# HilaManor/AudioEditingCode

Hardware: AMD Instinct MI355X
Metric: edited-clips/sec (200-step inv+edit, 10 s@16 kHz) (higher is better)
Workload: dtype f32

## Files before the change

audioeditingcode_amd/csrc/attention.hip:

```cpp
#include <mutex>
#include "aed_common.h"

typedef float f32x4 __attribute__((ext_vector_type(4)));

#include "attn_params.h"

#define KV_TILE 64
#define Q_TILE 64

template <int D>
__global__ __launch_bounds__(256) void attention_kernel(AttnParams p) {
    constexpr int KLD = D + 4;
    constexpr int VLD = KV_TILE + 4;
    constexpr int NB = D / 16;
    __shared__ __attribute__((aligned(16))) float Ks[KV_TILE * KLD];
    __shared__ __attribute__((aligned(16))) float Vt[D * VLD];
    __shared__ __attribute__((aligned(16))) float Ps[4 * 16 * VLD];

    const int tid = threadIdx.x;
    const int lane = tid & 63, wave = tid >> 6;
    const int fi = lane & 15, fh = lane >> 4;
    const int b = blockIdx.z, head = blockIdx.y;
    const int q0 = blockIdx.x * Q_TILE + wave * 16;
    const int hoff = head * D;

    const float* Q = p.q + (size_t)b * p.bsq + hoff;
    const float* K = p.k + (size_t)b * p.bsk + hoff;
    const float* V = p.v + (size_t)b * p.bsv + hoff;
    const float* bias = p.bias ? p.bias + (size_t)b * p.ld_bias : nullptr;

    float4 qf[NB];
    {
        const int qr = q0 + fi;
#pragma unroll
        for (int blk = 0; blk < NB; ++blk) {
            qf[blk] = make_float4(0.f, 0.f, 0.f, 0.f);
            if (qr < p.Nq) qf[blk] = *reinterpret_cast<const float4*>(Q + (size_t)qr * p.ldq + 16 * blk + 4 * fh);
        }
    }
    f32x4 oacc[NB];
#pragma unroll
    for (int c = 0; c < NB; ++c) oacc[c] = (f32x4){0.f, 0.f, 0.f, 0.f};
    float m_run[4], l_run[4];
#pragma unroll
    for (int r = 0; r < 4; ++r) { m_run[r] = -INFINITY; l_run[r] = 0.f; }

    float* Pw = Ps + wave * 16 * VLD;

    for (int k0 = 0; k0 < p.Nk; k0 += KV_TILE) {
        for (int idx = tid; idx < KV_TILE * (D / 4); idx += 256) {
            const int key = idx / (D / 4), c4 = idx - key * (D / 4);
            float4 v = make_float4(0.f, 0.f, 0.f, 0.f);
            if (k0 + key < p.Nk) v = *reinterpret_cast<const float4*>(K + (size_t)(k0 + key) * p.ldk + 4 * c4);
            *reinterpret_cast<float4*>(Ks + key * KLD + 4 * c4) = v;
        }
        {
            const int key = tid & 63, dg = tid >> 6;
            for (int dd = dg * 4; dd < D; dd += 16) {
                float4 v = make_float4(0.f, 0.f, 0.f, 0.f);
                if (k0 + key < p.Nk) v = *reinterpret_cast<const float4*>(V + (size_t)(k0 + key) * p.ldv + dd);
                Vt[(dd + 0) * VLD + key] = v.x;
                Vt[(dd + 1) * VLD + key] = v.y;
                Vt[(dd + 2) * VLD + key] = v.z;
                Vt[(dd + 3) * VLD + key] = v.w;
            }
        }
        __syncthreads();

        f32x4 sacc[4];
#pragma unroll
        for (int j = 0; j < 4; ++j) sacc[j] = (f32x4){0.f, 0.f, 0.f, 0.f};
#pragma unroll
        for (int blk = 0; blk < NB; ++blk) {
#pragma unroll
            for (int j = 0; j < 4; ++j) {
                const float4 kf = *reinterpret_cast<const float4*>(Ks + (16 * j + fi) * KLD + 16 * blk + 4 * fh);
                sacc[j] = __builtin_amdgcn_mfma_f32_16x16x4f32(qf[blk].x, kf.x, sacc[j], 0, 0, 0);
                sacc[j] = __builtin_amdgcn_mfma_f32_16x16x4f32(qf[blk].y, kf.y, sacc[j], 0, 0, 0);
                sacc[j] = __builtin_amdgcn_mfma_f32_16x16x4f32(qf[blk].z, kf.z, sacc[j], 0, 0, 0);
                sacc[j] = __builtin_amdgcn_mfma_f32_16x16x4f32(qf[blk].w, kf.w, sacc[j], 0, 0, 0);
            }
        }
        float tmax[4];
#pragma unroll
        for (int r = 0; r < 4; ++r) tmax[r] = -INFINITY;
#pragma unroll
        for (int j = 0; j < 4; ++j) {
            const int key = k0 + 16 * j + fi;
            const bool ok = key < p.Nk;
            const float bv = (ok && bias) ? bias[key] : 0.f;
#pragma unroll
            for (int r = 0; r < 4; ++r) {
                float s = ok ? sacc[j][r] * p.scale + bv : -INFINITY;
                sacc[j][r] = s;
                tmax[r] = fmaxf(tmax[r], s);
            }
        }
#pragma unroll
        for (int r = 0; r < 4; ++r) {
#pragma unroll
            for (int o = 8; o > 0; o >>= 1) tmax[r] = fmaxf(tmax[r], __shfl_xor(tmax[r], o, 16));
        }
        float alpha[4], rsum[4];
#pragma unroll
        for (int r = 0; r < 4; ++r) {
            const float mn = fmaxf(m_run[r], tmax[r]);
            alpha[r] = __expf(m_run[r] - mn);
            m_run[r] = mn;
            rsum[r] = 0.f;
        }
#pragma unroll
        for (int j = 0; j < 4; ++j) {
#pragma unroll
            for (int r = 0; r < 4; ++r) {
                const float pv = __expf(sacc[j][r] - m_run[r]);
                rsum[r] += pv;
                Pw[(4 * fh + r) * VLD + 16 * j + fi] = pv;
            }
        }
#pragma unroll
        for (int r = 0; r < 4; ++r) {
#pragma unroll
            for (int o = 8; o > 0; o >>= 1) rsum[r] += __shfl_xor(rsum[r], o, 16);
            l_run[r] = l_run[r] * alpha[r] + rsum[r];
        }
#pragma unroll
        for (int c = 0; c < NB; ++c)
#pragma unroll
            for (int r = 0; r < 4; ++r) oacc[c][r] *= alpha[r];

        __builtin_amdgcn_fence(__ATOMIC_ACQ_REL, "wavefront");
        __builtin_amdgcn_wave_barrier();

#pragma unroll
        for (int kb = 0; kb < 4; ++kb) {
            const float4 pf = *reinterpret_cast<const float4*>(Pw + fi * VLD + 16 * kb + 4 * fh);
#pragma unroll
            for (int c = 0; c < NB; ++c) {
                const float4 vf = *reinterpret_cast<const float4*>(Vt + (16 * c + fi) * VLD + 16 * kb + 4 * fh);
                oacc[c] = __builtin_amdgcn_mfma_f32_16x16x4f32(pf.x, vf.x, oacc[c], 0, 0, 0);
                oacc[c] = __builtin_amdgcn_mfma_f32_16x16x4f32(pf.y, vf.y, oacc[c], 0, 0, 0);
                oacc[c] = __builtin_amdgcn_mfma_f32_16x16x4f32(pf.z, vf.z, oacc[c], 0, 0, 0);
                oacc[c] = __builtin_amdgcn_mfma_f32_16x16x4f32(pf.w, vf.w, oacc[c], 0, 0, 0);
            }
        }
        __syncthreads();
    }

    float* O = p.o + (size_t)b * p.bso + hoff;
#pragma unroll
    for (int r = 0; r < 4; ++r) {
        const int qr = q0 + 4 * fh + r;
        if (qr >= p.Nq) continue;
        const float inv = 1.0f / l_run[r];
#pragma unroll
        for (int c = 0; c < NB; ++c) O[(size_t)qr * p.ldo + 16 * c + fi] = oacc[c][r] * inv;
    }
}

typedef float f32x16a __attribute__((ext_vector_type(16)));

template <int D, int KSPLIT>
__global__ __launch_bounds__(256) void attention_t_kernel(AttnParams p) {
    constexpr int DT = (D + 31) / 32;
    constexpr int KLD = D + 4;
    constexpr int VLD = 32 + 4;
    constexpr int NJ = D / 8;
    constexpr int SLAB = 32 * KLD + DT * 32 * VLD;
    constexpr int MSZ = DT * 16 + 2;
    static_assert(D % 8 == 0, "head dim");
    extern __shared__ __attribute__((aligned(16))) float smem[];
    const int tid = threadIdx.x, lane = tid & 63, wave = tid >> 6;
    const int fi = lane & 31, fh = lane >> 5;
    float* Ks = smem + wave * SLAB;
    float* Vt = Ks + 32 * KLD;

    int qt, head, b;
    {
        const unsigned nx = gridDim.x, ny = gridDim.y, nwg = nx * ny * gridDim.z;
        const unsigned orig = blockIdx.x + nx * (blockIdx.y + ny * blockIdx.z);
        const unsigned xcd = orig & 7u, q = nwg >> 3, r = nwg & 7u;
        const unsigned id = (xcd < r ? xcd * (q + 1) : r * (q + 1) + (xcd - r) * q) + (orig >> 3);
        qt = (int)(id % nx);
        head = (int)((id / nx) % ny);
        b = (int)(id / (nx * ny));
    }
    const int q0 = (KSPLIT == 1 ? qt * 128 + wave * 32 : qt * 32);
    const int hoff = head * D;
    const float* Q = p.q + (size_t)b * p.bsq + hoff;
    const float* K = p.k + (size_t)b * p.bsk + hoff;
    const float* V = p.v + (size_t)b * p.bsv + hoff;
    const float* bias = p.bias ? p.bias + (size_t)b * p.ld_bias : nullptr;

    float4 qf[NJ];
    {
        const int qr = min(q0 + fi, p.Nq - 1);
#pragma unroll
        for (int j = 0; j < NJ; ++j) {
            float4 v = *reinterpret_cast<const float4*>(Q + (size_t)qr * p.ldq + 8 * j + 4 * fh);
            qf[j] = make_float4(v.x * p.scale, v.y * p.scale, v.z * p.scale, v.w * p.scale);
        }
    }
    f32x16a oacc[DT];
#pragma unroll
    for (int c = 0; c < DT; ++c)
#pragma unroll
        for (int r = 0; r < 16; ++r) oacc[c][r] = 0.f;
    float m_run = -INFINITY, l_run = 0.f;

    constexpr int KC4 = D / 4;
    constexpr int NKL = (32 * KC4) / 64;
    float4 kreg[NKL], vreg[NKL];
    const int ntiles = (p.Nk + 31) / 32;
    auto prefetch = [&](int t) {
        const int k0 = min(t, ntiles - 1) * 32;
#pragma unroll
        for (int i = 0; i < NKL; ++i) {
            const int idx = lane + 64 * i;
            const int key = min(k0 + idx / KC4, p.Nk - 1);
            kreg[i] = *reinterpret_cast<const float4*>(K + (size_t)key * p.ldk + 4 * (idx % KC4));
        }
        const int vk = min(k0 + fi, p.Nk - 1);
#pragma unroll
        for (int i = 0; i < NKL; ++i)
            vreg[i] = *reinterpret_cast<const float4*>(V + (size_t)vk * p.ldv + 4 * (2 * i + fh));
    };
    auto stage = [&]() {
#pragma unroll
        for (int i = 0; i < NKL; ++i) {
            const int idx = lane + 64 * i;
            const float4 v = kreg[i];
            *reinterpret_cast<float4*>(Ks + (idx / KC4) * KLD + 4 * (idx % KC4)) = make_float4(v.x, v.y, v.z, v.w);
        }
#pragma unroll
        for (int i = 0; i < NKL; ++i) {
            const int dd = 4 * (2 * i + fh);
            const float4 v = vreg[i];
            Vt[(dd + 0) * VLD + fi] = v.x;
            Vt[(dd + 1) * VLD + fi] = v.y;
            Vt[(dd + 2) * VLD + fi] = v.z;
            Vt[(dd + 3) * VLD + fi] = v.w;
        }
    };
    if constexpr (DT * 32 > D) {
        for (int e = lane; e < (DT * 32 - D) * VLD; e += 64) Vt[D * VLD + e] = 0.f;
    }

    const int t_first = (KSPLIT == 1 ? 0 : wave);
    constexpr int TSTEP = (KSPLIT == 1 ? 1 : KSPLIT);
    prefetch(t_first);
    for (int t = t_first; t < ntiles; t += TSTEP) {
        stage();
        prefetch(t + TSTEP);
        asm volatile("" ::: "memory");
        __builtin_amdgcn_wave_barrier();
        f32x16a sacc;
#pragma unroll
        for (int r = 0; r < 16; ++r) sacc[r] = 0.f;
#pragma unroll
        for (int j = 0; j < NJ; ++j) {
            const float4 kf = *reinterpret_cast<const float4*>(Ks + fi * KLD + 8 * j + 4 * fh);
            sacc = __builtin_amdgcn_mfma_f32_32x32x2f32(kf.x, qf[j].x, sacc, 0, 0, 0);
            sacc = __builtin_amdgcn_mfma_f32_32x32x2f32(kf.y, qf[j].y, sacc, 0, 0, 0);
            sacc = __builtin_amdgcn_mfma_f32_32x32x2f32(kf.z, qf[j].z, sacc, 0, 0, 0);
            sacc = __builtin_amdgcn_mfma_f32_32x32x2f32(kf.w, qf[j].w, sacc, 0, 0, 0);
        }
        const int k0 = t * 32;
        if (bias) {
#pragma unroll
            for (int rq = 0; rq < 4; ++rq)
#pragma unroll
                for (int e = 0; e < 4; ++e)
                    sacc[4 * rq + e] += bias[min(k0 + 8 * rq + 4 * fh + e, p.Nk - 1)];
        }
        if (k0 + 32 > p.Nk) {
#pragma unroll
            for (int r = 0; r < 16; ++r)
                if (k0 + (r & 3) + 8 * (r >> 2) + 4 * fh >= p.Nk) sacc[r] = -INFINITY;
        }
        float mx = sacc[0];
#pragma unroll
        for (int r = 1; r < 16; ++r) mx = fmaxf(mx, sacc[r]);
        {
            auto sw = __builtin_amdgcn_permlane32_swap(__float_as_uint(mx), __float_as_uint(mx), false, false);
            mx = fmaxf(__uint_as_float(sw[0]), __uint_as_float(sw[1]));
        }
        const float mn = fmaxf(m_run, mx);
        const float alpha = __expf(m_run - mn);
        m_run = mn;
        float rsum = 0.f;
#pragma unroll
        for (int r = 0; r < 16; ++r) {
            sacc[r] = __expf(sacc[r] - mn);
            rsum += sacc[r];
        }
        l_run = l_run * alpha + rsum;
#pragma unroll
        for (int c = 0; c < DT; ++c)
#pragma unroll
            for (int r = 0; r < 16; ++r) oacc[c][r] *= alpha;
#pragma unroll
        for (int rq = 0; rq < 4; ++rq) {
#pragma unroll
            for (int c = 0; c < DT; ++c) {
                const float4 vf = *reinterpret_cast<const float4*>(Vt + (c * 32 + fi) * VLD + 8 * rq + 4 * fh);
                oacc[c] = __builtin_amdgcn_mfma_f32_32x32x2f32(vf.x, sacc[4 * rq + 0], oacc[c], 0, 0, 0);
                oacc[c] = __builtin_amdgcn_mfma_f32_32x32x2f32(vf.y, sacc[4 * rq + 1], oacc[c], 0, 0, 0);
                oacc[c] = __builtin_amdgcn_mfma_f32_32x32x2f32(vf.z, sacc[4 * rq + 2], oacc[c], 0, 0, 0);
                oacc[c] = __builtin_amdgcn_mfma_f32_32x32x2f32(vf.w, sacc[4 * rq + 3], oacc[c], 0, 0, 0);
            }
        }
        asm volatile("" ::: "memory");
        __builtin_amdgcn_wave_barrier();
    }

    if constexpr (KSPLIT > 1) {
        __syncthreads();
        float* mrg = smem;
        if (wave > 0) {
            float* dst = mrg + ((wave - 1) * 64 + lane) * MSZ;
            dst[0] = m_run;
            dst[1] = l_run;
#pragma unroll
            for (int c = 0; c < DT; ++c)
#pragma unroll
                for (int r = 0; r < 16; ++r) dst[2 + 16 * c + r] = oacc[c][r];
        }
        __syncthreads();
        if (wave > 0) return;
        float mt = m_run;
#pragma unroll
        for (int w = 0; w < KSPLIT - 1; ++w) mt = fmaxf(mt, mrg[(w * 64 + lane) * MSZ]);
        const float a0 = (m_run == -INFINITY) ? 0.f : __expf(m_run - mt);
        l_run *= a0;
#pragma unroll
        for (int c = 0; c < DT; ++c)
#pragma unroll
            for (int r = 0; r < 16; ++r) oacc[c][r] *= a0;
#pragma unroll
        for (int w = 0; w < KSPLIT - 1; ++w) {
            const float* src = mrg + (w * 64 + lane) * MSZ;
            const float mw = src[0];
            const float aw = (mw == -INFINITY) ? 0.f : __expf(mw - mt);
            l_run += src[1] * aw;
#pragma unroll
            for (int c = 0; c < DT; ++c)
#pragma unroll
                for (int r = 0; r < 16; ++r) oacc[c][r] += src[2 + 16 * c + r] * aw;
        }
    }
    {
        auto sw = __builtin_amdgcn_permlane32_swap(__float_as_uint(l_run), __float_as_uint(l_run), false, false);
        l_run = __uint_as_float(sw[0]) + __uint_as_float(sw[1]);
    }
    const float inv = 1.0f / l_run;
    const int qr = q0 + fi;
    if (qr < p.Nq) {
        float* O = p.o + (size_t)b * p.bso + hoff + (size_t)qr * p.ldo;
#pragma unroll
        for (int c = 0; c < DT; ++c)
#pragma unroll
            for (int rq = 0; rq < 4; ++rq) {
                const int d0 = c * 32 + 8 * rq + 4 * fh;
                if (d0 < D)
                    *reinterpret_cast<float4*>(O + d0) = make_float4(oacc[c][4 * rq] * inv, oacc[c][4 * rq + 1] * inv,
                                                                     oacc[c][4 * rq + 2] * inv, oacc[c][4 * rq + 3] * inv);
            }
    }
}

template <int D, int KSPLIT>
static int launch_t(const AttnParams& p, int B, hipStream_t s) {
    constexpr int DT = (D + 31) / 32;
    constexpr int SLAB = 32 * (D + 4) + DT * 32 * 36;
    constexpr int MRG = (KSPLIT - 1) * 64 * (DT * 16 + 2);
    const size_t bytes = sizeof(float) * (4 * SLAB > MRG ? 4 * SLAB : MRG);
    static std::once_flag attr_once;
    static hipError_t attr_rc = hipSuccess;
    std::call_once(attr_once, [&] {
        attr_rc = hipFuncSetAttribute((const void*)attention_t_kernel<D, KSPLIT>,
                                      hipFuncAttributeMaxDynamicSharedMemorySize, (int)bytes);
    });
    AED_CHECK_HIP(attr_rc);
    dim3 grid(aed_cdiv(p.Nq, KSPLIT == 1 ? 128 : 32), p.H, B);
    hipLaunchKernelGGL((attention_t_kernel<D, KSPLIT>), grid, dim3(256), bytes, s, p);
    return 0;
}

int launch_attention(const aed_op* op, hipStream_t s) {
    const int32_t* i = op->i;
    AttnParams p;
    p.q = (const float*)op->p[0]; p.k = (const float*)op->p[1]; p.v = (const float*)op->p[2];
    p.bias = (const float*)op->p[3]; p.o = (float*)op->p[4];
    AED_REQUIRE(p.q && p.k && p.v && p.o, "attention: null pointer");
    p.H = i[1]; p.Nq = i[2]; p.Nk = i[3];
    p.ldq = i[5]; p.ldk = i[6]; p.ldv = i[7]; p.ldo = i[8]; p.ld_bias = i[9];
    p.bsq = i[10]; p.bsk = i[11]; p.bsv = i[12]; p.bso = i[13];
    p.scale = op->f[0];
    AED_REQUIRE(p.ldq % 4 == 0 && p.ldk % 4 == 0 && p.ldv % 4 == 0, "attention: row strides must be multiples of 4");
    AED_REQUIRE(p.Nq > 0 && p.Nk > 0, "attention: empty sequence");
    AED_REQUIRE(p.ldo % 4 == 0, "attention: output row stride must be a multiple of 4");
    if (p.Nk > KV_TILE && i[14] != 1) {
        const long wg_ksplit1 = (long)aed_cdiv(p.Nq, 128) * p.H * i[0];
        const bool ks4 = wg_ksplit1 < 2L * aed_num_cus();
        int rc = 0;
        if (((op->flags & 4) && !ks4) || i[14] == 3) {
            rc = launch_attention_x6(p, i[0], i[4], s);
            if (rc >= 0) return rc;
            AED_REQUIRE(i[14] != 3, "attention: the split-bf16 kernel does not take head dim %d / these operands", i[4]);
        }
        switch (i[4]) {
            case 32: rc = ks4 ? launch_t<32, 4>(p, i[0], s) : launch_t<32, 1>(p, i[0], s); break;
            case 48: rc = ks4 ? launch_t<48, 4>(p, i[0], s) : launch_t<48, 1>(p, i[0], s); break;
            case 64: rc = ks4 ? launch_t<64, 4>(p, i[0], s) : launch_t<64, 1>(p, i[0], s); break;
            case 80: rc = ks4 ? launch_t<80, 4>(p, i[0], s) : launch_t<80, 1>(p, i[0], s); break;
            case 16: rc = ks4 ? launch_t<16, 4>(p, i[0], s) : launch_t<16, 1>(p, i[0], s); break;
            default: AED_REQUIRE(false, "attention: unsupported head dim %d (16/32/48/64/80)", i[4]);
        }
        if (rc) return rc;
        AED_CHECK_HIP(hipGetLastError());
        return 0;
    }
    dim3 grid(aed_cdiv(p.Nq, Q_TILE), p.H, i[0]);
    switch (i[4]) {
        case 16: hipLaunchKernelGGL(attention_kernel<16>, grid, dim3(256), 0, s, p); break;
        case 32: hipLaunchKernelGGL(attention_kernel<32>, grid, dim3(256), 0, s, p); break;
        case 48: hipLaunchKernelGGL(attention_kernel<48>, grid, dim3(256), 0, s, p); break;
        case 64: hipLaunchKernelGGL(attention_kernel<64>, grid, dim3(256), 0, s, p); break;
        case 80: hipLaunchKernelGGL(attention_kernel<80>, grid, dim3(256), 0, s, p); break;
        default: AED_REQUIRE(false, "attention: unsupported head dim %d (16/32/48/64/80)", i[4]);
    }
    AED_CHECK_HIP(hipGetLastError());
    return 0;
}
```

audioeditingcode_amd/csrc/attention_x6.hip:

```cpp
#include "attn_params.h"

typedef __bf16 abf16x8 __attribute__((ext_vector_type(8)));
typedef __bf16 abf16x2 __attribute__((ext_vector_type(2)));
typedef float af32x2 __attribute__((ext_vector_type(2)));
typedef float af32x16 __attribute__((ext_vector_type(16)));

__device__ __forceinline__ void ax6_split_pair(float x0, float x1, unsigned& h, unsigned& m, unsigned& l) {
    h = __builtin_bit_cast(unsigned, __builtin_convertvector((af32x2){x0, x1}, abf16x2));
    float r0 = x0 - __uint_as_float(h << 16);
    float r1 = x1 - __uint_as_float(h & 0xffff0000u);
    asm volatile("" : "+v"(r0), "+v"(r1));
    m = __builtin_bit_cast(unsigned, __builtin_convertvector((af32x2){r0, r1}, abf16x2));
    float q0 = r0 - __uint_as_float(m << 16);
    float q1 = r1 - __uint_as_float(m & 0xffff0000u);
    asm volatile("" : "+v"(q0), "+v"(q1));
    l = __builtin_bit_cast(unsigned, __builtin_convertvector((af32x2){q0, q1}, abf16x2));
}

__device__ __forceinline__ void ax6_split8(const float (&x)[8], abf16x8 (&f)[3]) {
    uint4 h, m, l;
    ax6_split_pair(x[0], x[1], h.x, m.x, l.x);
    ax6_split_pair(x[2], x[3], h.y, m.y, l.y);
    ax6_split_pair(x[4], x[5], h.z, m.z, l.z);
    ax6_split_pair(x[6], x[7], h.w, m.w, l.w);
    f[0] = __builtin_bit_cast(abf16x8, h);
    f[1] = __builtin_bit_cast(abf16x8, m);
    f[2] = __builtin_bit_cast(abf16x8, l);
}

__device__ __forceinline__ void ax6_mfma6(af32x16& acc, const abf16x8 (&a)[3], const abf16x8 (&b)[3]) {
    acc = __builtin_amdgcn_mfma_f32_32x32x16_bf16(a[0], b[2], acc, 0, 0, 0);
    acc = __builtin_amdgcn_mfma_f32_32x32x16_bf16(a[2], b[0], acc, 0, 0, 0);
    acc = __builtin_amdgcn_mfma_f32_32x32x16_bf16(a[1], b[1], acc, 0, 0, 0);
    acc = __builtin_amdgcn_mfma_f32_32x32x16_bf16(a[0], b[1], acc, 0, 0, 0);
    acc = __builtin_amdgcn_mfma_f32_32x32x16_bf16(a[1], b[0], acc, 0, 0, 0);
    acc = __builtin_amdgcn_mfma_f32_32x32x16_bf16(a[0], b[0], acc, 0, 0, 0);
}

template <int D>
__global__ __launch_bounds__(256, 2) void attention_x6_kernel(AttnParams p) {
    constexpr int NDB = D / 16;
    constexpr int DT = (D + 31) / 32;
    constexpr int KQ = NDB * 3 * 64;
    constexpr int VQ = 2 * 3 * DT * 64;
    constexpr int STAGE = KQ + VQ;
    constexpr int C4 = D / 4;
    constexpr int NK = (8 * D + 255) / 256;
    constexpr int NV = (8 * D + 255) / 256;
    static_assert(D % 16 == 0 && 2 * STAGE * 16 <= 65536, "head dim");
    __shared__ uint4 lds[2 * STAGE];

    const int tid = threadIdx.x, lane = tid & 63, wave = tid >> 6;
    const int fi = lane & 31, fh = lane >> 5;
    int qt, head, b;
    {
        const unsigned nx = gridDim.x, ny = gridDim.y, nwg = nx * ny * gridDim.z;
        const unsigned orig = blockIdx.x + nx * (blockIdx.y + ny * blockIdx.z);
        const unsigned xcd = orig & 7u, q = nwg >> 3, r = nwg & 7u;
        const unsigned id = (xcd < r ? xcd * (q + 1) : r * (q + 1) + (xcd - r) * q) + (orig >> 3);
        qt = (int)(id % nx);
        head = (int)((id / nx) % ny);
        b = (int)(id / (nx * ny));
    }
    const int q0 = qt * 128 + wave * 32;
    const int hoff = head * D;
    const float* Q = p.q + (size_t)b * p.bsq + hoff;
    const float* K = p.k + (size_t)b * p.bsk + hoff;
    const float* V = p.v + (size_t)b * p.bsv + hoff;
    const float* bias = p.bias ? p.bias + (size_t)b * p.ld_bias : nullptr;

    abf16x8 qp[NDB][3];
    {
        const float* qrow = Q + (size_t)min(q0 + fi, p.Nq - 1) * p.ldq + 8 * fh;
#pragma unroll
        for (int db = 0; db < NDB; ++db) {
            const float4 a = *reinterpret_cast<const float4*>(qrow + 16 * db);
            const float4 c = *reinterpret_cast<const float4*>(qrow + 16 * db + 4);
            const float x[8] = {a.x * p.scale, a.y * p.scale, a.z * p.scale, a.w * p.scale,
                                c.x * p.scale, c.y * p.scale, c.z * p.scale, c.w * p.scale};
            ax6_split8(x, qp[db]);
        }
    }
    af32x16 oacc[DT];
#pragma unroll
    for (int c = 0; c < DT; ++c)
#pragma unroll
        for (int r = 0; r < 16; ++r) oacc[c][r] = 0.f;
    float m_run = -INFINITY, l_run = 0.f;

    const int ntiles = (p.Nk + 31) / 32;
    float4 kreg[2][NK];
    float vreg[2][NV][4];
    auto prefetch = [&](int t, float4 (&kr)[NK], float (&vr)[NV][4]) {
        const int k0 = min(t, ntiles - 1) * 32;
#pragma unroll
        for (int i = 0; i < NK; ++i) {
            const int item = min(tid + 256 * i, 8 * D - 1);
            const int key = min(k0 + item / C4, p.Nk - 1);
            kr[i] = *reinterpret_cast<const float4*>(K + (size_t)key * p.ldk + 4 * (item % C4));
        }
#pragma unroll
        for (int i = 0; i < NV; ++i) {
            const int item = min(tid + 256 * i, 8 * D - 1);
            const int kg = item / D, d = item - kg * D;
#pragma unroll
            for (int j = 0; j < 4; ++j)
                vr[i][j] = V[(size_t)min(k0 + 4 * kg + j, p.Nk - 1) * p.ldv + d];
        }
    };
    auto stage_write = [&](uint4* st, const float4 (&kr)[NK], const float (&vr)[NV][4]) {
        uint2* k2 = reinterpret_cast<uint2*>(st);
        uint2* v2 = reinterpret_cast<uint2*>(st + KQ);
#pragma unroll
        for (int i = 0; i < NK; ++i) {
            const int item = tid + 256 * i;
            if (8 * D % 256 != 0 && item >= 8 * D) break;
            const int key = item / C4, c4 = item % C4;
            unsigned h0, m0, l0, h1, m1, l1;
            ax6_split_pair(kr[i].x, kr[i].y, h0, m0, l0);
            ax6_split_pair(kr[i].z, kr[i].w, h1, m1, l1);
            uint2* dst = k2 + ((c4 >> 2) * 3 * 32 + key) * 4 + ((c4 >> 1) & 1) * 2 + (c4 & 1);
            dst[0] = make_uint2(h0, h1);
            dst[32 * 4] = make_uint2(m0, m1);
            dst[2 * 32 * 4] = make_uint2(l0, l1);
        }
#pragma unroll
        for (int i = 0; i < NV; ++i) {
            const int item = tid + 256 * i;
            if (8 * D % 256 != 0 && item >= 8 * D) break;
            const int kg = item / D, d = item - kg * D;
            unsigned h0, m0, l0, h1, m1, l1;
            ax6_split_pair(vr[i][0], vr[i][1], h0, m0, l0);
            ax6_split_pair(vr[i][2], vr[i][3], h1, m1, l1);
            const int kb = kg >> 2, g = kg & 3;
            uint2* dst = v2 + (((kb * 3) * DT + (d >> 5)) * 32 + (d & 31)) * 4 + (g & 1) * 2 + (g >> 1);
            dst[0] = make_uint2(h0, h1);
            dst[DT * 32 * 4] = make_uint2(m0, m1);
            dst[2 * DT * 32 * 4] = make_uint2(l0, l1);
        }
    };
    if constexpr (DT * 32 > D) {
        for (int e = tid; e < 2 * STAGE; e += 256) lds[e] = make_uint4(0u, 0u, 0u, 0u);
        __syncthreads();
    }

    prefetch(0, kreg[0], vreg[0]);
    prefetch(1, kreg[1], vreg[1]);
    stage_write(lds, kreg[0], vreg[0]);
    prefetch(2, kreg[0], vreg[0]);
    __syncthreads();
    for (int t0 = 0; t0 < ntiles; t0 += 2) {
#pragma unroll
        for (int u = 0; u < 2; ++u) {
            const int t = t0 + u;
            const uint4* st = lds + u * STAGE;
            af32x16 sacc;
#pragma unroll
            for (int r = 0; r < 16; ++r) sacc[r] = 0.f;
#pragma unroll
            for (int db = 0; db < NDB; ++db) {
                abf16x8 kf[3];
#pragma unroll
                for (int pl = 0; pl < 3; ++pl) kf[pl] = __builtin_bit_cast(abf16x8, st[((db * 3 + pl) * 32 + fi) * 2 + fh]);
                ax6_mfma6(sacc, kf, qp[db]);
            }
            stage_write(lds + (u ^ 1) * STAGE, kreg[u ^ 1], vreg[u ^ 1]);
            prefetch(t + 3, kreg[u ^ 1], vreg[u ^ 1]);
            const int k0 = t * 32;
            if (bias) {
#pragma unroll
                for (int rq = 0; rq < 4; ++rq)
#pragma unroll
                    for (int e = 0; e < 4; ++e)
                        sacc[4 * rq + e] += bias[min(k0 + 8 * rq + 4 * fh + e, p.Nk - 1)];
            }
            if (k0 + 32 > p.Nk) {
#pragma unroll
                for (int r = 0; r < 16; ++r)
                    if (k0 + (r & 3) + 8 * (r >> 2) + 4 * fh >= p.Nk) sacc[r] = -INFINITY;
            }
            float mx = sacc[0];
#pragma unroll
            for (int r = 1; r < 16; ++r) mx = fmaxf(mx, sacc[r]);
            {
                auto sw = __builtin_amdgcn_permlane32_swap(__float_as_uint(mx), __float_as_uint(mx), false, false);
                mx = fmaxf(__uint_as_float(sw[0]), __uint_as_float(sw[1]));
            }
            const float mn = fmaxf(m_run, mx);
            const float alpha = __expf(m_run - mn);
            m_run = mn;
            float rsum = 0.f;
#pragma unroll
            for (int r = 0; r < 16; ++r) {
                sacc[r] = __expf(sacc[r] - mn);
                rsum += sacc[r];
            }
            l_run = l_run * alpha + rsum;
#pragma unroll
            for (int c = 0; c < DT; ++c)
#pragma unroll
                for (int r = 0; r < 16; ++r) oacc[c][r] *= alpha;
#pragma unroll
            for (int kb = 0; kb < 2; ++kb) {
                abf16x8 pf[3];
                const float x[8] = {sacc[8 * kb], sacc[8 * kb + 1], sacc[8 * kb + 2], sacc[8 * kb + 3],
                                    sacc[8 * kb + 4], sacc[8 * kb + 5], sacc[8 * kb + 6], sacc[8 * kb + 7]};
                ax6_split8(x, pf);
#pragma unroll
                for (int c = 0; c < DT; ++c) {
                    abf16x8 vf[3];
#pragma unroll
                    for (int pl = 0; pl < 3; ++pl)
                        vf[pl] = __builtin_bit_cast(abf16x8, st[KQ + (((kb * 3 + pl) * DT + c) * 32 + fi) * 2 + fh]);
                    ax6_mfma6(oacc[c], vf, pf);
                }
            }
            __syncthreads();
        }
    }

    {
        auto sw = __builtin_amdgcn_permlane32_swap(__float_as_uint(l_run), __float_as_uint(l_run), false, false);
        l_run = __uint_as_float(sw[0]) + __uint_as_float(sw[1]);
    }
    const float inv = 1.0f / l_run;
    const int qr = q0 + fi;
    if (qr < p.Nq) {
        float* O = p.o + (size_t)b * p.bso + hoff + (size_t)qr * p.ldo;
#pragma unroll
        for (int c = 0; c < DT; ++c)
#pragma unroll
            for (int rq = 0; rq < 4; ++rq) {
                const int d0 = c * 32 + 8 * rq + 4 * fh;
                if (d0 < D)
                    *reinterpret_cast<float4*>(O + d0) = make_float4(oacc[c][4 * rq] * inv, oacc[c][4 * rq + 1] * inv,
                                                                     oacc[c][4 * rq + 2] * inv, oacc[c][4 * rq + 3] * inv);
            }
    }
}

template <int D>
static int launch_ax6(const AttnParams& p, int B, hipStream_t s) {
    dim3 grid(aed_cdiv(p.Nq, 128), p.H, B);
    hipLaunchKernelGGL((attention_x6_kernel<D>), grid, dim3(256), 0, s, p);
    AED_CHECK_HIP(hipGetLastError());
    return 0;
}

int launch_attention_x6(const AttnParams& p, int B, int D, hipStream_t s) {
    if (((uintptr_t)p.q | (uintptr_t)p.k) % 16 != 0) return -1;
    switch (D) {
        case 32: return launch_ax6<32>(p, B, s);
        case 48: return launch_ax6<48>(p, B, s);
        case 64: return launch_ax6<64>(p, B, s);
        default: return -1;
    }
}
```

audioeditingcode_amd/csrc/attn_params.h:

```cpp
#pragma once
#include "aed_common.h"

struct AttnParams {
    const float* q; const float* k; const float* v; const float* bias; float* o;
    int Nq, Nk, H;
    int ldq, ldk, ldv, ldo, ld_bias;
    long bsq, bsk, bsv, bso;
    float scale;
};

int launch_attention_x6(const AttnParams& p, int B, int D, hipStream_t s);
```

Measured before the change: 0.9084.

## Software-pipeline split-bf16 attention: overlap next-tile QK MFMAs with softmax

Restructures the split-bf16 attention kernel so the QK^T MFMAs for the next KV tile are interleaved with the softmax, rescaling, P splitting and K staging of the current tile. It uses compile-time unrolled placement with sched_group_barrier hints. It also precomputes 32-bit byte offsets for K/V prefetch, specializes the kernel on bias presence, and keeps the old serial schedule selectable through a mode flag. The aim is to hide exp/VALU and LDS latency behind matrix-core work, at the cost of higher register pressure and offsets that are limited to strides below 2^24.

```diff
diff --git a/audioeditingcode_amd/csrc/attention.hip b/audioeditingcode_amd/csrc/attention.hip
--- a/audioeditingcode_amd/csrc/attention.hip
+++ b/audioeditingcode_amd/csrc/attention.hip
@@ -400,14 +400,14 @@
     AED_REQUIRE(p.ldq % 4 == 0 && p.ldk % 4 == 0 && p.ldv % 4 == 0, "attention: row strides must be multiples of 4");
     AED_REQUIRE(p.Nq > 0 && p.Nk > 0, "attention: empty sequence");
     AED_REQUIRE(p.ldo % 4 == 0, "attention: output row stride must be a multiple of 4");
-    if (p.Nk > KV_TILE && i[14] != 1) {
+    if ((p.Nk > KV_TILE || i[14] >= 3) && i[14] != 1) {
         const long wg_ksplit1 = (long)aed_cdiv(p.Nq, 128) * p.H * i[0];
         const bool ks4 = wg_ksplit1 < 2L * aed_num_cus();
         int rc = 0;
-        if (((op->flags & 4) && !ks4) || i[14] == 3) {
-            rc = launch_attention_x6(p, i[0], i[4], s);
+        if (((op->flags & 4) && !ks4) || i[14] >= 3) {
+            rc = launch_attention_x6(p, i[0], i[4], i[14] == 4, s);
             if (rc >= 0) return rc;
-            AED_REQUIRE(i[14] != 3, "attention: the split-bf16 kernel does not take head dim %d / these operands", i[4]);
+            AED_REQUIRE(i[14] < 3, "attention: the split-bf16 kernel does not take head dim %d / these operands", i[4]);
         }
         switch (i[4]) {
             case 32: rc = ks4 ? launch_t<32, 4>(p, i[0], s) : launch_t<32, 1>(p, i[0], s); break;
diff --git a/audioeditingcode_amd/csrc/attention_x6.hip b/audioeditingcode_amd/csrc/attention_x6.hip
--- a/audioeditingcode_amd/csrc/attention_x6.hip
+++ b/audioeditingcode_amd/csrc/attention_x6.hip
@@ -1,4 +1,5 @@
 #include "attn_params.h"
+#include <type_traits>
 
 typedef __bf16 abf16x8 __attribute__((ext_vector_type(8)));
 typedef __bf16 abf16x2 __attribute__((ext_vector_type(2)));
@@ -37,7 +38,32 @@
     acc = __builtin_amdgcn_mfma_f32_32x32x16_bf16(a[0], b[0], acc, 0, 0, 0);
 }
 
-template <int D>
+template <int I, int N, class F>
+__device__ __forceinline__ void ax6_static_for(F&& f) {
+    if constexpr (I < N) {
+        f(std::integral_constant<int, I>{});
+        ax6_static_for<I + 1, N>(f);
+    }
+}
+
+template <int T>
+__device__ __forceinline__ void ax6_mfma1(af32x16& acc, const abf16x8 (&a)[3], const abf16x8 (&b)[3]) {
+    constexpr int TA[6] = {0, 2, 1, 0, 1, 0};
+    constexpr int TB[6] = {2, 0, 1, 1, 0, 0};
+    acc = __builtin_amdgcn_mfma_f32_32x32x16_bf16(a[TA[T]], b[TB[T]], acc, 0, 0, 0);
+}
+
+template <int G, int NM, int NV>
+__device__ __forceinline__ void ax6_hints() {
+    if constexpr (G < NM) {
+        constexpr int v = (NV * (G + 1)) / NM - (NV * G) / NM;
+        if constexpr (v > 0) __builtin_amdgcn_sched_group_barrier(0x002, v, 0);
+        __builtin_amdgcn_sched_group_barrier(0x008, 1, 0);
+        ax6_hints<G + 1, NM, NV>();
+    }
+}
+
+template <int D, bool PIPE, bool BIAS>
 __global__ __launch_bounds__(256, 2) void attention_x6_kernel(AttnParams p) {
     constexpr int NDB = D / 16;
     constexpr int DT = (D + 31) / 32;
@@ -48,6 +74,7 @@
     constexpr int NK = (8 * D + 255) / 256;
     constexpr int NV = (8 * D + 255) / 256;
     static_assert(D % 16 == 0 && 2 * STAGE * 16 <= 65536, "head dim");
+    constexpr int HV2 = 48, HV3 = 26 * NV;
     __shared__ uint4 lds[2 * STAGE];
 
     const int tid = threadIdx.x, lane = tid & 63, wave = tid >> 6;
@@ -91,39 +118,86 @@
     const int ntiles = (p.Nk + 31) / 32;
     float4 kreg[2][NK];
     float vreg[2][NV][4];
-    auto prefetch = [&](int t, float4 (&kr)[NK], float (&vr)[NV][4]) {
-        const int k0 = min(t, ntiles - 1) * 32;
+    unsigned koff[NK], koff_last[NK], voff[NV][4], voff_last[NV][4];
+    const int last_rows = p.Nk - 1 - (ntiles - 1) * 32;
+    if constexpr (PIPE) {
 #pragma unroll
         for (int i = 0; i < NK; ++i) {
             const int item = min(tid + 256 * i, 8 * D - 1);
-            const int key = min(k0 + item / C4, p.Nk - 1);
-            kr[i] = *reinterpret_cast<const float4*>(K + (size_t)key * p.ldk + 4 * (item % C4));
+            const int row = item / C4, col = 4 * (item % C4);
+            koff[i] = 4u * (unsigned)(row * p.ldk + col);
+            koff_last[i] = 4u * (unsigned)(min(row, last_rows) * p.ldk + col);
         }
 #pragma unroll
         for (int i = 0; i < NV; ++i) {
             const int item = min(tid + 256 * i, 8 * D - 1);
             const int kg = item / D, d = item - kg * D;
 #pragma unroll
-            for (int j = 0; j < 4; ++j)
-                vr[i][j] = V[(size_t)min(k0 + 4 * kg + j, p.Nk - 1) * p.ldv + d];
-        }
-    };
-    auto stage_write = [&](uint4* st, const float4 (&kr)[NK], const float (&vr)[NV][4]) {
+            for (int j = 0; j < 4; ++j) {
+                voff[i][j] = 4u * (unsigned)((4 * kg + j) * p.ldv + d);
+                voff_last[i][j] = 4u * (unsigned)(min(4 * kg + j, last_rows) * p.ldv + d);
+            }
+        }
+    }
+    auto prefetch_k = [&](int t, float4 (&kr)[NK]) {
+        const int tc = min(t, ntiles - 1);
+        if constexpr (PIPE) {
+            const char* base = reinterpret_cast<const char*>(K + (size_t)tc * 32 * p.ldk);
+            const bool last = tc == ntiles - 1;
+#pragma unroll
+            for (int i = 0; i < NK; ++i)
+                kr[i] = *reinterpret_cast<const float4*>(base + (last ? koff_last[i] : koff[i]));
+        } else {
+            const int k0 = tc * 32;
+#pragma unroll
+            for (int i = 0; i < NK; ++i) {
+                const int item = min(tid + 256 * i, 8 * D - 1);
+                const int key = min(k0 + item / C4, p.Nk - 1);
+                kr[i] = *reinterpret_cast<const float4*>(K + (size_t)key * p.ldk + 4 * (item % C4));
+            }
+        }
+    };
+    auto prefetch_v = [&](int t, float (&vr)[NV][4]) {
+        const int tc = min(t, ntiles - 1);
+        if constexpr (PIPE) {
+            const char* base = reinterpret_cast<const char*>(V + (size_t)tc * 32 * p.ldv);
+            const bool last = tc == ntiles - 1;
+#pragma unroll
+            for (int i = 0; i < NV; ++i)
+#pragma unroll
+                for (int j = 0; j < 4; ++j)
+                    vr[i][j] = *reinterpret_cast<const float*>(base + (last ? voff_last[i][j] : voff[i][j]));
+        } else {
+            const int k0 = tc * 32;
+#pragma unroll
+            for (int i = 0; i < NV; ++i) {
+                const int item = min(tid + 256 * i, 8 * D - 1);
+                const int kg = item / D, d = item - kg * D;
+#pragma unroll
+                for (int j = 0; j < 4; ++j)
+                    vr[i][j] = V[(size_t)min(k0 + 4 * kg + j, p.Nk - 1) * p.ldv + d];
+            }
+        }
+    };
+    auto stage_write_k_item = [&](uint4* st, const float4 (&kr)[NK], int i) {
         uint2* k2 = reinterpret_cast<uint2*>(st);
+        const int item = tid + 256 * i;
+        if (8 * D % 256 != 0 && item >= 8 * D) return;
+        const int key = item / C4, c4 = item % C4;
+        unsigned h0, m0, l0, h1, m1, l1;
+        ax6_split_pair(kr[i].x, kr[i].y, h0, m0, l0);
+        ax6_split_pair(kr[i].z, kr[i].w, h1, m1, l1);
+        uint2* dst = k2 + ((c4 >> 2) * 3 * 32 + key) * 4 + ((c4 >> 1) & 1) * 2 + (c4 & 1);
+        dst[0] = make_uint2(h0, h1);
+        dst[32 * 4] = make_uint2(m0, m1);
+        dst[2 * 32 * 4] = make_uint2(l0, l1);
+    };
+    auto stage_write_k = [&](uint4* st, const float4 (&kr)[NK]) {
+#pragma unroll
+        for (int i = 0; i < NK; ++i) stage_write_k_item(st, kr, i);
+    };
+    auto stage_write_v = [&](uint4* st, const float (&vr)[NV][4]) {
         uint2* v2 = reinterpret_cast<uint2*>(st + KQ);
-#pragma unroll
-        for (int i = 0; i < NK; ++i) {
-            const int item = tid + 256 * i;
-            if (8 * D % 256 != 0 && item >= 8 * D) break;
-            const int key = item / C4, c4 = item % C4;
-            unsigned h0, m0, l0, h1, m1, l1;
-            ax6_split_pair(kr[i].x, kr[i].y, h0, m0, l0);
-            ax6_split_pair(kr[i].z, kr[i].w, h1, m1, l1);
-            uint2* dst = k2 + ((c4 >> 2) * 3 * 32 + key) * 4 + ((c4 >> 1) & 1) * 2 + (c4 & 1);
-            dst[0] = make_uint2(h0, h1);
-            dst[32 * 4] = make_uint2(m0, m1);
-            dst[2 * 32 * 4] = make_uint2(l0, l1);
-        }
 #pragma unroll
         for (int i = 0; i < NV; ++i) {
             const int item = tid + 256 * i;
@@ -144,79 +218,212 @@
         __syncthreads();
     }
 
-    prefetch(0, kreg[0], vreg[0]);
-    prefetch(1, kreg[1], vreg[1]);
-    stage_write(lds, kreg[0], vreg[0]);
-    prefetch(2, kreg[0], vreg[0]);
-    __syncthreads();
-    for (int t0 = 0; t0 < ntiles; t0 += 2) {
-#pragma unroll
-        for (int u = 0; u < 2; ++u) {
-            const int t = t0 + u;
-            const uint4* st = lds + u * STAGE;
-            af32x16 sacc;
-#pragma unroll
-            for (int r = 0; r < 16; ++r) sacc[r] = 0.f;
-#pragma unroll
-            for (int db = 0; db < NDB; ++db) {
-                abf16x8 kf[3];
-#pragma unroll
-                for (int pl = 0; pl < 3; ++pl) kf[pl] = __builtin_bit_cast(abf16x8, st[((db * 3 + pl) * 32 + fi) * 2 + fh]);
-                ax6_mfma6(sacc, kf, qp[db]);
-            }
-            stage_write(lds + (u ^ 1) * STAGE, kreg[u ^ 1], vreg[u ^ 1]);
-            prefetch(t + 3, kreg[u ^ 1], vreg[u ^ 1]);
-            const int k0 = t * 32;
-            if (bias) {
-#pragma unroll
-                for (int rq = 0; rq < 4; ++rq)
-#pragma unroll
-                    for (int e = 0; e < 4; ++e)
-                        sacc[4 * rq + e] += bias[min(k0 + 8 * rq + 4 * fh + e, p.Nk - 1)];
-            }
-            if (k0 + 32 > p.Nk) {
-#pragma unroll
-                for (int r = 0; r < 16; ++r)
-                    if (k0 + (r & 3) + 8 * (r >> 2) + 4 * fh >= p.Nk) sacc[r] = -INFINITY;
-            }
-            float mx = sacc[0];
-#pragma unroll
-            for (int r = 1; r < 16; ++r) mx = fmaxf(mx, sacc[r]);
-            {
-                auto sw = __builtin_amdgcn_permlane32_swap(__float_as_uint(mx), __float_as_uint(mx), false, false);
-                mx = fmaxf(__uint_as_float(sw[0]), __uint_as_float(sw[1]));
-            }
-            const float mn = fmaxf(m_run, mx);
-            const float alpha = __expf(m_run - mn);
-            m_run = mn;
-            float rsum = 0.f;
-#pragma unroll
-            for (int r = 0; r < 16; ++r) {
-                sacc[r] = __expf(sacc[r] - mn);
-                rsum += sacc[r];
-            }
-            l_run = l_run * alpha + rsum;
-#pragma unroll
-            for (int c = 0; c < DT; ++c)
-#pragma unroll
-                for (int r = 0; r < 16; ++r) oacc[c][r] *= alpha;
-#pragma unroll
-            for (int kb = 0; kb < 2; ++kb) {
-                abf16x8 pf[3];
-                const float x[8] = {sacc[8 * kb], sacc[8 * kb + 1], sacc[8 * kb + 2], sacc[8 * kb + 3],
-                                    sacc[8 * kb + 4], sacc[8 * kb + 5], sacc[8 * kb + 6], sacc[8 * kb + 7]};
-                ax6_split8(x, pf);
-#pragma unroll
-                for (int c = 0; c < DT; ++c) {
-                    abf16x8 vf[3];
+    auto scores = [&](af32x16& sacc, const uint4* st) {
+#pragma unroll
+        for (int r = 0; r < 16; ++r) sacc[r] = 0.f;
+#pragma unroll
+        for (int db = 0; db < NDB; ++db) {
+            abf16x8 kf[3];
+#pragma unroll
+            for (int pl = 0; pl < 3; ++pl) kf[pl] = __builtin_bit_cast(abf16x8, st[((db * 3 + pl) * 32 + fi) * 2 + fh]);
+            ax6_mfma6(sacc, kf, qp[db]);
+        }
+    };
+    auto softmax = [&](int t, af32x16& sacc, auto has_bias, auto ragged) {
+        const int k0 = t * 32;
+        if (has_bias) {
+#pragma unroll
+            for (int rq = 0; rq < 4; ++rq)
+#pragma unroll
+                for (int e = 0; e < 4; ++e)
+                    sacc[4 * rq + e] += bias[min(k0 + 8 * rq + 4 * fh + e, p.Nk - 1)];
+        }
+        if (ragged && k0 + 32 > p.Nk) {
+#pragma unroll
+            for (int r = 0; r < 16; ++r)
+                if (k0 + (r & 3) + 8 * (r >> 2) + 4 * fh >= p.Nk) sacc[r] = -INFINITY;
+        }
+        float mx = sacc[0];
+#pragma unroll
+        for (int r = 1; r < 16; ++r) mx = fmaxf(mx, sacc[r]);
+        {
+            auto sw = __builtin_amdgcn_permlane32_swap(__float_as_uint(mx), __float_as_uint(mx), false, false);
+            mx = fmaxf(__uint_as_float(sw[0]), __uint_as_float(sw[1]));
+        }
+        const float mn = fmaxf(m_run, mx);
+        const float alpha = __expf(m_run - mn);
+        m_run = mn;
+        float rsum = 0.f;
+#pragma unroll
+        for (int r = 0; r < 16; ++r) {
+            sacc[r] = __expf(sacc[r] - mn);
+            rsum += sacc[r];
+        }
+        l_run = l_run * alpha + rsum;
+#pragma unroll
+        for (int c = 0; c < DT; ++c)
+#pragma unroll
+            for (int r = 0; r < 16; ++r) oacc[c][r] *= alpha;
+    };
+    auto split_p = [&](const af32x16& sacc, int kb, abf16x8 (&pf)[3]) {
+        const float x[8] = {sacc[8 * kb], sacc[8 * kb + 1], sacc[8 * kb + 2], sacc[8 * kb + 3],
+                            sacc[8 * kb + 4], sacc[8 * kb + 5], sacc[8 * kb + 6], sacc[8 * kb + 7]};
+        ax6_split8(x, pf);
+    };
+    auto read_v = [&](const uint4* st, int kb, abf16x8 (&vf)[DT][3]) {
+#pragma unroll
+        for (int c = 0; c < DT; ++c)
+#pragma unroll
+            for (int pl = 0; pl < 3; ++pl)
+                vf[c][pl] = __builtin_bit_cast(abf16x8, st[KQ + (((kb * 3 + pl) * DT + c) * 32 + fi) * 2 + fh]);
+    };
+    auto pv = [&](const abf16x8 (&vf)[DT][3], const abf16x8 (&pf)[3]) {
+#pragma unroll
+        for (int c = 0; c < DT; ++c) ax6_mfma6(oacc[c], vf[c], pf);
+    };
+
+    if constexpr (!PIPE) {
+        prefetch_k(0, kreg[0]);
+        prefetch_v(0, vreg[0]);
+        prefetch_k(1, kreg[1]);
+        prefetch_v(1, vreg[1]);
+        stage_write_k(lds, kreg[0]);
+        stage_write_v(lds, vreg[0]);
+        prefetch_k(2, kreg[0]);
+        prefetch_v(2, vreg[0]);
+        __syncthreads();
+        for (int t0 = 0; t0 < ntiles; t0 += 2) {
+#pragma unroll
+            for (int u = 0; u < 2; ++u) {
+                const int t = t0 + u;
+                const uint4* st = lds + u * STAGE;
+                af32x16 sacc;
+                scores(sacc, st);
+                stage_write_k(lds + (u ^ 1) * STAGE, kreg[u ^ 1]);
+                stage_write_v(lds + (u ^ 1) * STAGE, vreg[u ^ 1]);
+                prefetch_k(t + 3, kreg[u ^ 1]);
+                prefetch_v(t + 3, vreg[u ^ 1]);
+                softmax(t, sacc, bias != nullptr, std::true_type{});
+#pragma unroll
+                for (int kb = 0; kb < 2; ++kb) {
+                    abf16x8 pf[3], vf[DT][3];
+                    split_p(sacc, kb, pf);
+                    read_v(st, kb, vf);
+                    pv(vf, pf);
+                }
+                __syncthreads();
+            }
+        }
+    } else {
+        prefetch_k(0, kreg[0]);
+        prefetch_k(1, kreg[1]);
+        prefetch_v(0, vreg[0]);
+        prefetch_v(1, vreg[1]);
+        stage_write_k(lds, kreg[0]);
+        prefetch_k(2, kreg[0]);
+        stage_write_k(lds + STAGE, kreg[1]);
+        prefetch_k(3, kreg[1]);
+        stage_write_v(lds, vreg[0]);
+        prefetch_v(2, vreg[0]);
+        __syncthreads();
+        af32x16 s_even, s_odd;
+        scores(s_even, lds);
+        __syncthreads();
+        auto tile = [&](int t, auto uc, af32x16& cur, af32x16& nxt, auto edge, auto next) {
+            constexpr int u = decltype(uc)::value;
+            constexpr bool hint = !decltype(edge)::value;
+            abf16x8 pf0[3], pf1[3], vf0[DT][3], vf1[DT][3];
+            if constexpr (!hint) {
+                if (next) scores(nxt, lds + (u ^ 1) * STAGE);
+                softmax(t, cur, std::bool_constant<BIAS>{}, edge);
+                split_p(cur, 0, pf0);
+                stage_write_k(lds + u * STAGE, kreg[u]);
+            } else {
+                constexpr int NM = 6 * NDB, U_EXP = 1, U_RES = 9, U_SPL = U_RES + 2 * DT, U_K = U_SPL + 4, NU = U_K + NK;
+                const uint4* kst = lds + (u ^ 1) * STAGE;
+                abf16x8 kf[NDB][3];
+#pragma unroll
+                for (int db = 0; db < NDB; ++db)
 #pragma unroll
                     for (int pl = 0; pl < 3; ++pl)
-                        vf[pl] = __builtin_bit_cast(abf16x8, st[KQ + (((kb * 3 + pl) * DT + c) * 32 + fi) * 2 + fh]);
-                    ax6_mfma6(oacc[c], vf, pf);
-                }
-            }
+                        kf[db][pl] = __builtin_bit_cast(abf16x8, kst[((db * 3 + pl) * 32 + fi) * 2 + fh]);
+#pragma unroll
+                for (int r = 0; r < 16; ++r) nxt[r] = 0.f;
+                float mn, alpha, rsum = 0.f;
+                uint4 ph, pm, pl4;
+                unsigned* const phw = reinterpret_cast<unsigned*>(&ph);
+                ax6_static_for<0, NM>([&](auto ic) {
+                    constexpr int i = decltype(ic)::value;
+                    ax6_mfma1<i % 6>(nxt, kf[i / 6], qp[i / 6]);
+                    ax6_static_for<0, NU>([&](auto jc) {
+                        constexpr int j = decltype(jc)::value;
+                        if constexpr (j * NM / NU == i) {
+                            if constexpr (j == 0) {
+                                if constexpr (BIAS) {
+                                    const int k0 = t * 32;
+#pragma unroll
+                                    for (int rq = 0; rq < 4; ++rq)
+#pragma unroll
+                                        for (int e = 0; e < 4; ++e)
+                                            cur[4 * rq + e] += bias[min(k0 + 8 * rq + 4 * fh + e, p.Nk - 1)];
+                                }
+                                float mx = cur[0];
+#pragma unroll
+                                for (int r = 1; r < 16; ++r) mx = fmaxf(mx, cur[r]);
+                                auto sw = __builtin_amdgcn_permlane32_swap(__float_as_uint(mx), __float_as_uint(mx), false, false);
+                                mx = fmaxf(__uint_as_float(sw[0]), __uint_as_float(sw[1]));
+                                mn = fmaxf(m_run, mx);
+                                alpha = __expf(m_run - mn);
+                                m_run = mn;
+                            } else if constexpr (j < U_RES) {
+#pragma unroll
+                                for (int r = 2 * (j - U_EXP); r < 2 * (j - U_EXP) + 2; ++r) {
+                                    cur[r] = __expf(cur[r] - mn);
+                                    rsum += cur[r];
+                                }
+                                if constexpr (j == U_RES - 1) l_run = l_run * alpha + rsum;
+                            } else if constexpr (j < U_SPL) {
+#pragma unroll
+                                for (int r = 8 * ((j - U_RES) & 1); r < 8 * ((j - U_RES) & 1) + 8; ++r) oacc[(j - U_RES) >> 1][r] *= alpha;
+                            } else if constexpr (j < U_K) {
+                                constexpr int q = j - U_SPL;
+                                ax6_split_pair(cur[2 * q], cur[2 * q + 1], phw[q], reinterpret_cast<unsigned*>(&pm)[q],
+                                               reinterpret_cast<unsigned*>(&pl4)[q]);
+                            } else {
+                                stage_write_k_item(lds + u * STAGE, kreg[u], j - U_K);
+                            }
+                        }
+                    });
+                    __builtin_amdgcn_sched_barrier(0);
+                });
+                pf0[0] = __builtin_bit_cast(abf16x8, ph);
+                pf0[1] = __builtin_bit_cast(abf16x8, pm);
+                pf0[2] = __builtin_bit_cast(abf16x8, pl4);
+            }
+            read_v(lds + u * STAGE, 0, vf0);
+            __builtin_amdgcn_sched_barrier(0);
+            pv(vf0, pf0);
+            split_p(cur, 1, pf1);
+            prefetch_k(t + 4, kreg[u]);
+            read_v(lds + u * STAGE, 1, vf1);
+            if constexpr (hint) ax6_hints<0, 6 * DT, HV2>();
+            __builtin_amdgcn_sched_barrier(0);
+            pv(vf1, pf1);
+            stage_write_v(lds + (u ^ 1) * STAGE, vreg[u ^ 1]);
+            prefetch_v(t + 3, vreg[u ^ 1]);
+            if constexpr (hint) ax6_hints<0, 6 * DT, HV3>();
             __syncthreads();
-        }
+            __builtin_amdgcn_sched_barrier(0);
+        };
+        using U0 = std::integral_constant<int, 0>;
+        using U1 = std::integral_constant<int, 1>;
+        int t0 = 0;
+        for (; t0 + 2 < ntiles; t0 += 2) {
+            tile(t0, U0{}, s_even, s_odd, std::false_type{}, std::true_type{});
+            tile(t0 + 1, U1{}, s_odd, s_even, std::false_type{}, std::true_type{});
+        }
+        tile(t0, U0{}, s_even, s_odd, std::true_type{}, std::true_type{});
+        tile(t0 + 1, U1{}, s_odd, s_even, std::true_type{}, std::false_type{});
     }
 
     {
@@ -240,19 +447,22 @@
 }
 
 template <int D>
-static int launch_ax6(const AttnParams& p, int B, hipStream_t s) {
+static int launch_ax6(const AttnParams& p, int B, bool serial, hipStream_t s) {
     dim3 grid(aed_cdiv(p.Nq, 128), p.H, B);
-    hipLaunchKernelGGL((attention_x6_kernel<D>), grid, dim3(256), 0, s, p);
+    if (serial) hipLaunchKernelGGL((attention_x6_kernel<D, false, false>), grid, dim3(256), 0, s, p);
+    else if (p.bias) hipLaunchKernelGGL((attention_x6_kernel<D, true, true>), grid, dim3(256), 0, s, p);
+    else hipLaunchKernelGGL((attention_x6_kernel<D, true, false>), grid, dim3(256), 0, s, p);
     AED_CHECK_HIP(hipGetLastError());
     return 0;
 }
 
-int launch_attention_x6(const AttnParams& p, int B, int D, hipStream_t s) {
+int launch_attention_x6(const AttnParams& p, int B, int D, bool serial, hipStream_t s) {
     if (((uintptr_t)p.q | (uintptr_t)p.k) % 16 != 0) return -1;
+    if (p.ldk >= (1 << 24) || p.ldv >= (1 << 24)) return -1;
     switch (D) {
-        case 32: return launch_ax6<32>(p, B, s);
-        case 48: return launch_ax6<48>(p, B, s);
-        case 64: return launch_ax6<64>(p, B, s);
+        case 32: return launch_ax6<32>(p, B, serial, s);
+        case 48: return launch_ax6<48>(p, B, serial, s);
+        case 64: return launch_ax6<64>(p, B, serial, s);
         default: return -1;
     }
 }
diff --git a/audioeditingcode_amd/csrc/attn_params.h b/audioeditingcode_amd/csrc/attn_params.h
--- a/audioeditingcode_amd/csrc/attn_params.h
+++ b/audioeditingcode_amd/csrc/attn_params.h
@@ -9,4 +9,4 @@
     float scale;
 };
 
-int launch_attention_x6(const AttnParams& p, int B, int D, hipStream_t s);
+int launch_attention_x6(const AttnParams& p, int B, int D, bool serial, hipStream_t s);
```

Result: no change. 0.9143, median of 6 (+0.6%).
